# dkogan/horizonator

Hardware: AMD Instinct MI355X
Metric: panorama Mpix/s (360deg, 16k-wide, 7x7 SRTM3 tiles) (higher is better)
Workload: dtype f32

## Files before the change

### horizonator_amd/_lib.py

```python
import ctypes as C
import os

_HERE = os.path.dirname(os.path.abspath(__file__))
LIB_PATH = os.environ.get("HORIZONATOR_AMD_LIB") or os.path.join(_HERE, "libhorizonator.so")
DEMGEN_PATH = os.path.join(_HERE, "libhzdemgen.so")
SELFTEST_PATH = os.path.join(_HERE, "libhorizonator_selftest.so")

MAX_NDEMS_IJ = 4


class DemContext(C.Structure):
    _fields_ = [
        ("dems", (C.c_void_p * MAX_NDEMS_IJ) * MAX_NDEMS_IJ),
        ("mmap_sizes", (C.c_size_t * MAX_NDEMS_IJ) * MAX_NDEMS_IJ),
        ("mmap_fd", (C.c_int * MAX_NDEMS_IJ) * MAX_NDEMS_IJ),
        ("origin_dem_lon_lat", C.c_int * 2),
        ("origin_dem_cellij", C.c_int * 2),
        ("Ndems_ij", C.c_int * 2),
        ("radius_cells", C.c_int),
        ("cells_per_deg", C.c_int),
    ]


class _Offscreen(C.Structure):
# ... 166 lines not shown
    sig("hz_hip_last_times", i, vp, P(Times))
    sig("hz_hip_stream", vp, vp)
    sig("hz_hip_wait_outputs", i, vp, vp)
    sig("hz_hip_wait_for", i, vp, vp)
    sig("horizonator_amd_stream_waits_for_outputs", b, ctxp, vp)
    sig("horizonator_amd_waits_for_stream", b, ctxp, vp)
    sig("hz_hip_last_plan", i, vp, vp)
    sig("hz_hip_last_queue_counts", i, vp, vp)
    sig("hz_hip_last_error", C.c_char_p)
    if selftest:
        sig("hz_hip_check_fastmath", i, i, i, C.c_uint64, C.c_uint64, P(C.c_uint64), vp)
        sig("hz_hip_check_exactness", i, i, i, C.c_uint64, C.c_uint64, i, i, i, i, P(C.c_uint64))
        sig("hz_hip_debug_bigqueue", i, vp, i, vp, i, vp)
        sig("hz_hip_debug_wave_timing", i, vp, P(View), vp, C.c_size_t, vp)
        sig("hz_hip_debug_worklist", C.c_long, i, i, i, P(View), i, i, i, vp, C.c_size_t)
    return lib


DECLARED_SYMBOLS = [
    "horizonator_init", "horizonator_deinit", "horizonator_resized", "horizonator_pan_zoom",
    "horizonator_move", "horizonator_set_zextents", "horizonator_redraw", "horizonator_pick",
    "horizonator_render_offscreen", "horizonator_x_from_az", "horizonator_project",
    "horizonator_unproject",
    "horizonator_dem_init", "horizonator_dem_deinit", "horizonator_dem_sample",
    "horizonator_dem_bounds_latlon_deg",
    "horizonator_amd_get_window", "horizonator_amd_init_from_mosaic",
    "horizonator_amd_render", "horizonator_amd_render_device", "horizonator_amd_render_batch",
    "horizonator_amd_render_packed", "horizonator_amd_resolve_packed",
    "horizonator_amd_resolve_packed_strips", "horizonator_amd_render_sparse",
    "horizonator_amd_resolve_sparse_strips",
    "horizonator_amd_sync", "horizonator_amd_stream_waits_for_outputs", "horizonator_amd_waits_for_stream", "horizonator_amd_texture_layout", "horizonator_amd_set_texture",
    "horizonator_amd_set_sector", "horizonator_amd_set_raster", "horizonator_amd_set_profiling",
    "horizonator_amd_get_options", "horizonator_amd_set_options", "horizonator_amd_render_begin", "horizonator_amd_render_end",
    "horizonator_amd_last_times", "horizonator_amd_get_view", "horizonator_amd_device",
    "horizonator_amd_get_mosaic", "horizonator_amd_link_cells_size", "horizonator_amd_link_cells",
    "horizonator_amd_poi_visibility", "horizonator_amd_build_id",
    "hz_hip_device_count", "hz_hip_create", "hz_hip_destroy", "hz_hip_upload_mosaic",
    "hz_hip_download_mosaic", "hz_hip_ingest_tiles", "hz_hip_set_sector", "hz_hip_set_raster",
    "hz_hip_set_profiling", "hz_hip_get_options", "hz_hip_set_options", "hz_hip_set_texture", "hz_hip_pack", "hz_hip_resolve_packed", "hz_hip_pack_sparse", "hz_hip_resolve_sparse", "hz_hip_resolve_sparse_strips", "hz_hip_draw", "hz_hip_resolve", "hz_hip_resolve_to_host", "hz_hip_render_to_host", "hz_hip_host_begin", "hz_hip_host_end", "hz_hip_host_prepare",
    "hz_hip_read_depth", "hz_hip_link_cells", "hz_hip_poi_visibility", "hz_hip_sync", "hz_hip_last_times", "hz_hip_stream", "hz_hip_wait_outputs", "hz_hip_wait_for", "hz_hip_last_plan", "hz_hip_last_queue_counts", "hz_hip_last_error",
]
SELFTEST_SYMBOLS = ["hz_hip_check_fastmath", "hz_hip_check_exactness", "hz_hip_debug_bigqueue", "hz_hip_debug_wave_timing",
                    "hz_hip_debug_worklist"]


def load_demgen():
    if not os.path.exists(DEMGEN_PATH):
        raise ImportError(f"{DEMGEN_PATH} is missing: build it with `make -C horizonator_amd/csrc`")
    lib = C.CDLL(DEMGEN_PATH)
    lib.hz_demgen_write_region.restype = C.c_int
    lib.hz_demgen_write_region.argtypes = [C.c_char_p] + [C.c_int] * 6
    lib.hz_demgen_write_tile.restype = C.c_int
    lib.hz_demgen_write_tile.argtypes = [C.c_char_p] + [C.c_int] * 4
    lib.hz_demgen_tile_values.restype = None
    lib.hz_demgen_tile_values.argtypes = [C.c_void_p] + [C.c_int] * 4
    return lib
```

### horizonator_amd/csrc/hz_context.cpp

```cpp
#include "hz_dev.h"

#include <time.h>

thread_local char hz_g_last_error[512];
extern "C" const char* hz_hip_last_error(void) { return g_last_error; }


static int env_int(const char* name, int dflt) { const char* e = getenv(name); return e ? atoi(e) : dflt; }
static hz_options_t default_options(void)
{
    hz_options_t o;
    o.serial         = 0;
    o.rounds         = 0;
    o.near_cells     = -1;
    o.coarse_depth   = -1;
    o.tiles          = -1;
    o.tile_list      = 0;
    o.adapt          = 1;
    o.adapt_hi       = -1;
    o.pretest_march  = -1;
    o.worklists      = 1;
    o.fast_math      = 1;
    o.resolve_clears = 1;
    o.queue_capacity = 0;
// ... 54 lines not shown
    hz_device_guard device_guard_(d->device);
    (void)hz_sync_all(d);
    (void)hipFree(d->d_mosaic);
    for(int i=0; i<HZ_NFB; i++) { (void)hipFree(d->d_fbs[i]); (void)hipFree(d->d_touched[i]); }
    for(int i=0; i<2*HZ_NFB; i++)
    {
        (void)hipFree(d->d_bigrec_s[i]);
        (void)hipFree(d->d_bigitem_s[i]);
        (void)hipFree(d->d_midrec_s[i]);
        (void)hipFree(d->d_clip_s[i]);
        (void)hipFree(d->d_big_counters_s[i]);
        (void)hipFree(d->tiles_s[i].cursor); (void)hipFree(d->tiles_s[i].pairs); (void)hipFree(d->tiles_s[i].state); (void)hipFree(d->tiles_s[i].busy);
    }
    if(d->ev_marched) (void)hipEventDestroy(d->ev_marched);
    if(d->ev_near)    (void)hipEventDestroy(d->ev_near);
    for(int i=0; i<HZ_NFB; i++) (void)hipFree(d->d_hiz[i]);
    for(int c=0; c<HZ_LIST_CACHE; c++)
        for(int k=0; k<HZ_NLISTS; k++)
        {
            hz_worklists_t& wl = d->list_cache[c];
            (void)hipFree(wl.d_items[k]);
            for(int t=0; t<2; t++)
            {
                if(wl.h_items[k][t])   (void)hipHostFree(wl.h_items[k][t]);
                if(wl.ev_copied[k][t]) (void)hipEventDestroy(wl.ev_copied[k][t]);
            }
        }
    delete d->list_scratch; delete d->list_scratch2;
    (void)hipFree(d->d_texels);
    (void)hipFree(d->d_tanel);
// ... 93 lines not shown
        d->near_bigrec_capacity  = near_tris < rec ? (unsigned int)near_tris : rec;
        d->near_bigitem_capacity = 2*rec;
        d->near_clip_capacity    = d->near_bigrec_capacity;
        if(d->env.queue_capacity > 0)
            d->bigrec_capacity = d->bigitem_capacity = d->midrec_capacity = d->clip_capacity =
            d->near_bigrec_capacity = d->near_bigitem_capacity = d->near_clip_capacity = (unsigned int)d->env.queue_capacity;
    }
    if(d->env.serial) d->qstream = d->nstream = d->stream;
    else
    {
        HZ_CHECK(hipStreamCreateWithFlags(&d->qstream, hipStreamNonBlocking));
        HZ_CHECK(hipStreamCreateWithFlags(&d->nstream, hipStreamNonBlocking));
    }
    HZ_CHECK(hipEventCreateWithFlags(&d->ev_marched, hipEventDisableTiming));
    HZ_CHECK(hipEventCreateWithFlags(&d->ev_near,    hipEventDisableTiming));
    for(int i=0; i<2*HZ_NFB; i++)
    {
        const mr_queue_t q = hz_queue_set(d, i);
        HZ_CHECK(hipMalloc(&d->d_bigrec_s[i],  (size_t)q.bigrec_capacity*sizeof(hz_bigrec_t)));
        HZ_CHECK(hipMalloc(&d->d_bigitem_s[i], (size_t)q.bigitem_capacity*sizeof(hz_bigitem_t)));
        if(q.midrec_capacity) HZ_CHECK(hipMalloc(&d->d_midrec_s[i], (size_t)q.midrec_capacity*sizeof(hz_rec_t)));
        HZ_CHECK(hipMalloc(&d->d_clip_s[i],    (size_t)q.clip_capacity*sizeof(uint32_t)));
        HZ_CHECK(hipMalloc(&d->d_big_counters_s[i], HZ_NCOUNTERS*sizeof(unsigned int)));
        HZ_CHECK(hipMemset(d->d_big_counters_s[i], 0, HZ_NCOUNTERS*sizeof(unsigned int)));
        if(d->env.tiles > 0 && i >= HZ_NFB && hz_tile_bins(d, i) != 0) return -1;
    }
    sw.lap("queue sets");
    HZ_CHECK(hipEventRecord(d->ev_drawn, d->qstream));
    HZ_CHECK(hipMalloc(&d->d_tanel, (size_t)d->H*sizeof(float)));
    d->h_tanel = (float*)malloc((size_t)d->H*sizeof(float));
    d->tanel_resident = 0;
    for(int k=0; k<10; k++) HZ_CHECK(hipEventCreate(&d->ev[k]));
    for(int k=0; k<HZ_NFB; k++)
    {
        HZ_CHECK(hipHostMalloc((void**)&d->adapt.h_counts[k], 6*sizeof(unsigned int), hipHostMallocDefault));
        HZ_CHECK(hipEventCreateWithFlags(&d->adapt.ev[k], hipEventDisableTiming | hipEventReleaseToSystem));
    }
    sw.lap("the rest");
    return 0;
// ... 172 lines not shown
```

### horizonator_amd/csrc/hz_dev.h

```cpp
#pragma once

#include <hip/hip_runtime_api.h>

#include <math.h>
#include <stdio.h>
#include <stdlib.h>
#include <string.h>
#include <time.h>

#include <vector>

#include "hz_hip.h"
#include "hz_types.h"
#include "hz_launch.h"


extern thread_local char hz_g_last_error[512];
#define g_last_error hz_g_last_error

#define HZ_CHECK(call)                                                        \
    do {                                                                      \
        hipError_t e_ = (call);                                               \
        if(e_ != hipSuccess)                                                  \
        {                                                                     \
// ... 65 lines not shown
    std::vector<uint32_t>* list_scratch;
    std::vector<uint32_t>* list_scratch2;
    struct { unsigned long long* d_cycles; size_t capacity; unsigned int grid_x, grid_y; } wave_timing;

    hipStream_t stream, rstream;
    hipEvent_t  ev_drawn, ev_free[HZ_NFB], ev_readers, ev_tanel;
    int16_t*            d_mosaic;
    unsigned long long* d_fbs[HZ_NFB];
    size_t              fb_used[HZ_NFB];
    int                 fbi;
    unsigned long long* d_fb;
    unsigned char*      d_touched[HZ_NFB];
    int                 seg_stride;
    hipStream_t         qstream, nstream;
    hipEvent_t          ev_marched, ev_near;
    uint32_t*           d_hiz[HZ_NFB];
    int                 hiz_unavailable;
    int                 tiles_unavailable;
    struct
    {
        unsigned int* h_counts[HZ_NFB];
        hipEvent_t    ev[HZ_NFB];
        int           pending[HZ_NFB], long_of[HZ_NFB], reach_of[HZ_NFB];
        unsigned int  serial_of[HZ_NFB];
        hz_view_t     view; int col0, col1, have_view;
        unsigned int  serial;
        unsigned int  items_short;
        int           tried_long;
        int           long_reach;
        int           seen_reach; unsigned int seen_records, seen_items;
    } adapt;
    struct { hz_polar_t* d_polar; hz_xform_t key; int state ; int unavailable; hipEvent_t ev_filled;
             int same_draw;      } vc;
    int                 last_qshards_log2;
    int                 last_plan[5];
    int                 stream_reads_fb;
    hz_bigrec_t*        d_bigrec_s[2*HZ_NFB];
    hz_bigitem_t*       d_bigitem_s[2*HZ_NFB];
    hz_rec_t*           d_midrec_s[2*HZ_NFB];
    uint32_t*           d_clip_s[2*HZ_NFB];
    unsigned int*       d_big_counters_s[2*HZ_NFB];
    unsigned int        bigrec_capacity, bigitem_capacity, midrec_capacity, clip_capacity;
    unsigned int        near_bigrec_capacity, near_bigitem_capacity, near_clip_capacity;
    tl_bins_t           tiles_s[2*HZ_NFB];
    hz_view_t           last_view;
    int                 have_view;
    int                 fb_consumed;
    float*              d_tanel;
    float*              h_tanel;
    int                 tanel_resident;

    struct hz_hoststate* host;

    uint32_t*      d_texels;
    hz_texparams_t tex;
    int            tex_on;
// ... 49 lines not shown
```

### horizonator_amd/csrc/hz_draw.cpp

```cpp
#include "hz_dev.h"
#include "hz_fast.h"

static int upload_list(hz_dev_t* d, int which, hipStream_t st, const std::vector<uint32_t>& items)
{
    hz_worklists_t& wl = *d->lists;
    const size_t n = items.size();
    if(n > wl.cap[which])
    {
        HZ_CHECK(hz_sync_all(d));
        (void)hipFree(wl.d_items[which]); wl.d_items[which] = NULL;
        for(int t=0; t<2; t++) { if(wl.h_items[which][t]) (void)hipHostFree(wl.h_items[which][t]); wl.h_items[which][t] = NULL; }
        wl.cap[which] = 0;
        const size_t cap = n + n/4 + 1024;
        hipError_t e = hipMalloc(&wl.d_items[which], cap*sizeof(uint32_t));
        for(int t=0; t<2 && e == hipSuccess; t++) e = hipHostMalloc((void**)&wl.h_items[which][t], cap*sizeof(uint32_t), hipHostMallocDefault);
        if(e != hipSuccess)
        {
            (void)hipFree(wl.d_items[which]); wl.d_items[which] = NULL;
            for(int t=0; t<2; t++) { if(wl.h_items[which][t]) (void)hipHostFree(wl.h_items[which][t]); wl.h_items[which][t] = NULL; }
            HZ_CHECK(e);
        }
        wl.cap[which] = cap;
    }
    const int t = wl.turn[which]; wl.turn[which] ^= 1;
// ... 158 lines not shown
                return 0;
            }
            HZ_CHECK(hipEventCreateWithFlags(&d->vc.ev_filled, hipEventDisableTiming));
        }
        HZ_CHECK(hipStreamWaitEvent(d->nstream, d->ev_marched, 0));
        hzk_polar_fill(dim3((unsigned)((d->N + 255)/256), 1024), dim3(256), d->nstream, (const int16_t*)d->d_mosaic, d->vc.d_polar, d->N, p.u);
        HZ_CHECK(hipGetLastError());
        HZ_CHECK(hipEventRecord(d->vc.ev_filled, d->nstream));
        HZ_CHECK(hipStreamWaitEvent(d->stream, d->vc.ev_filled, 0));
        d->vc.state = 2;
    }
    p.vcache = d->vc.d_polar;
    return 0;
}

int hz_draw_impl(hz_dev_t* d, const hz_view_t* view)
{
    hz_params_t p = hz_make_params(d, view);
    const bool prof = d->profiling != 0;
    d->last_view = *view; d->have_view = 1; d->fb_consumed = 0;
    if(!d->adapt.have_view || memcmp(view, &d->adapt.view, sizeof(*view)) != 0 || d->adapt.col0 != d->col0 || d->adapt.col1 != d->col1)
    {
        d->adapt.view = *view; d->adapt.col0 = d->col0; d->adapt.col1 = d->col1; d->adapt.have_view = 1;
        d->adapt.serial++; d->adapt.items_short = 0; d->adapt.tried_long = 0; d->adapt.long_reach = 0;
    }
    for(int k=0; k<HZ_NFB; k++)
        if(d->adapt.pending[k] && hipEventQuery(d->adapt.ev[k]) == hipSuccess)
        {
            d->adapt.pending[k] = 0;
            const unsigned int items = d->adapt.h_counts[k][1];
// ... 51 lines not shown
            {
                hz_worklists_t* e = &d->list_cache[c];
                if(e->valid && memcmp(&key, &e->key, sizeof(key)) == 0) { hit = e; break; }
                if((!e->valid && lru->valid) || (e->valid == lru->valid && e->last_used < lru->last_used)) lru = e;
            }
            fresh_lists = hit == NULL;
            d->lists = hit ? hit : lru;
            d->lists->last_used = ++d->lists_clock;
            if(fresh_lists) { d->lists->valid = 0; d->lists->key = key; }
        }
        if(two_pass)
        {
            p.inline_max = HZ_INLINE_MAX_PIX;
            const mr_queue_t qn = hz_queue_set(d, HZ_NFB + next);
            HZ_CHECK(hipStreamWaitEvent(d->nstream, d->ev_free[next], 0));
            {
                const float ppr = p.halfW * p.u.az_ndc_per_rad;
                const float reach = 0.5f*(float)(p.near_j1 - p.near_j0);
                zoomed_view = reach > 0.f && ppr/reach >= HZ_HIZ_MIN_PX;
                const float cells_to_zfar = view->zfar / (p.u.deg_per_cell * 111194.9f);
                p.qshards_log2 = (zoomed_view || cells_to_zfar <= 0.25f*ppr) ? HZ_QSHARDS_LOG2 : 0;
            }
            hz_params_t p1 = p;
            p1.pass = 1; p1.early_z = 0;
            if(fresh_lists)
            {
                hz_list_rounds(p1, zn, a0, a1, false, d->list_scratch, *d->list_scratch2);
                if(upload_list(d, 0, d->nstream, *d->list_scratch) != 0) return -1;
            }
            if(prof) HZ_CHECK(hipEventRecord(d->ev[7], d->nstream));
// ... 24 lines not shown
                HZ_CHECK(hipStreamWaitEvent(d->stream, d->ev_near, 0));
                waited_near = true;
            }
            else
                near_beside_far = true;
            p.pass = 2; p.early_z = early_z ? 1 : 0;
            {
                const float ppr = p.halfW * p.u.az_ndc_per_rad;
                const float cells_to_zfar = view->zfar / (p.u.deg_per_cell * 111194.9f);
                if(cells_to_zfar <= 0.25f*ppr) p.inline_max = 32;
            }
            p.hiz = hz.l1;
            p.pretest_march = d->env.pretest_march >= 0 ? d->env.pretest_march
                                                        : ((unsigned long long)p.SW*(unsigned long long)p.H*8ull > (256ull << 20) ? 1 : 0);
        }
        else if(prof) { HZ_CHECK(hipEventRecord(d->ev[7], d->stream)); HZ_CHECK(hipEventRecord(d->ev[6], d->stream)); }
        if(!waited_near) HZ_CHECK(hipStreamWaitEvent(d->stream, d->ev_free[next], 0));
        if(fresh_lists)
        {
            if(!two_pass) hz_list_rounds(p, zn, a0, a1, true, NULL, *d->list_scratch2);
            if(upload_list(d, 1, d->stream, *d->list_scratch2) != 0) return -1;
            d->lists->valid = 1;
        }
        if(prof) HZ_CHECK(hipEventRecord(d->ev[9], d->stream));
        if(launch_march(d, d->stream, q, zn, p, listed ? d->lists->d_items[1] : NULL, d->lists->n[1]) != 0) return -1;
    }
    if(prof) HZ_CHECK(hipEventRecord(d->ev[2], d->stream));
    HZ_CHECK(hipEventRecord(d->ev_marched, d->stream));
    HZ_CHECK(hipStreamWaitEvent(d->qstream, d->ev_marched, 0));
    if(near_beside_far) HZ_CHECK(hipStreamWaitEvent(d->qstream, d->ev_near, 0));
    if(prof) HZ_CHECK(hipEventRecord(d->ev[8], d->qstream));
    unsigned int* report = NULL;
// ... 38 lines not shown
```

### horizonator_amd/csrc/hz_fast.h

```cpp
#pragma once

#include "hz_num.h"

#ifdef __HIPCC__

#define HZF_LO 9.31322575e-10f
#define HZF_HI 1073741824.0f

__device__ static inline int hzf_in_range(float x) { const float a = hz_abs(x); return a >= HZF_LO && a <= HZF_HI; }

__device__ static inline float hzf_refined_rcp(float c)
{
    const float r = __builtin_amdgcn_rcpf(c);
    const float e = __builtin_fmaf(-c, r, 1.0f);
    return __builtin_fmaf(e, r, r);
}
__device__ static inline float hzf_div_by(float a, float c, float rr)
{
    float q = a*rr;
    float e = __builtin_fmaf(-c, q, a);
    q = __builtin_fmaf(e, rr, q);
    e = __builtin_fmaf(-c, q, a);
    return __builtin_fmaf(e, rr, q);
}
// ... 51 lines not shown
    p = p + u7*-0.1173503194786851f;
    p = p + u9*0.0536813784310406f;
    p = p + (u9*-0.0121323213173444f)*u2;
    const float a   = (1.0f < tn) ? ((p*-2.0f + HZ_HALF_PI) + p) : p;
    const float arc = flip ? (HZ_HALF_PI + a) : a;
    const uint32_t sign = ((uint32_t)__float_as_int(y) | (uint32_t)__float_as_int(rcp)) & 0x80000000u;
    return __int_as_float((int)((uint32_t)__float_as_int(arc) | sign));
}
template<bool XPOS>
__device__ static inline float hzf_atan2(float y, float x)
{
    const float t = (XPOS ? false : (0.f >= x)) ? y : hz_abs(x);
    return hzf_atan2_r<XPOS>(y, x, hzf_rcp(t));
}

__device__ static inline hz_polar_t hzf_polar_en_r(const hz_xform_t* u, float e, float n, float fz, float rcp_az)
{
    hz_polar_t q;
    const float h = fz - u->viewer_z;
    const float nn = n*n, ee = e*e;
    q.d_ne  = hzf_sqrt(nn + ee);
    q.az    = hzf_atan2_r<false>(e, n, rcp_az);
    q.el    = hzf_atan2<true>(h, q.d_ne);
    q.d_enh = hzf_sqrt(h*h + nn + ee);
    return q;
}
__device__ static inline hz_polar_t hzf_polar_en(const hz_xform_t* u, float e, float n, float fz)
{
    return hzf_polar_en_r(u, e, n, fz, hzf_rcp((0.f >= n) ? e : hz_abs(n)));
}
__device__ static inline hz_vertex_t hzf_finish(const hz_xform_t* u, const hzf_const_t* c, hz_polar_t q)
{
    hz_vertex_t v;
    const float d = hzf_div_by_two_pi(q.az + -u->az_center, c->rr_two_pi);
    v.x = (HZ_TWO_PI*(d - hz_roundeven(d))) * u->az_ndc_per_rad;
    v.y = q.el * u->aspect * u->az_ndc_per_rad;
    v.z = hzf_div_by(q.d_enh - u->znear, c->zrange, c->rr_zrange) * 2.0f + -1.0f;

    const float r = hzf_div_by(q.d_ne - u->znear_color, c->crange, c->rr_crange);
    v.red = hz_min(hz_max(r, 0.0f), 1.0f);
    return v;
}
__device__ static inline hz_vertex_t hzf_transform_en(const hz_xform_t* u, const hzf_const_t* c, float e, float n, float fz)
{
    return hzf_finish(u, c, hzf_polar_en(u, e, n, fz));
}
__device__ static inline hz_vertex_t hzf_transform_en_r(const hz_xform_t* u, const hzf_const_t* c, float e, float n, float fz, float rcp_az)
{
    return hzf_finish(u, c, hzf_polar_en_r(u, e, n, fz, rcp_az));
}

#endif

HZ_HD int hzf_draw_ok(const hz_xform_t* u)
{
    const float lo = 9.31322575e-10f, hi = 1073741824.0f;
    const float vz = hz_abs(u->viewer_z), ce = hz_abs(u->az_center);
    const float zr = hz_abs(u->zfar - u->znear), cr = hz_abs(u->zfar_color - u->znear_color);
    if(!(vz == 0.0f || (vz >= 0.015625f && vz <= 536870912.0f))) return 0;
    if(!(ce == 0.0f || (ce >= 8.8817842e-16f && ce <= 1048576.0f))) return 0;
    if(!(u->znear >= lo && u->znear <= hi && hz_abs(u->zfar) >= lo && hz_abs(u->zfar) <= hi && zr >= lo && zr <= hi)) return 0;
    if(!(hz_abs(u->znear_color) >= lo && hz_abs(u->znear_color) <= hi &&
         hz_abs(u->zfar_color) >= lo && hz_abs(u->zfar_color) <= hi && cr >= lo && cr <= hi)) return 0;
    if(!(hz_abs(u->aspect) <= hi && hz_abs(u->az_ndc_per_rad) <= hi)) return 0;
    return 1;
// ... 2 lines not shown
```

### horizonator_amd/csrc/hz_k_march.h

```cpp
#pragma once


#define MR_CAP    128
#define MR_RSLOTS 4
#define MR_FIELDS 6

struct mr_lds_t
{
    uint32_t rows[MR_RSLOTS][MR_FIELDS][64];
    uint32_t ids[MR_CAP];
    uint32_t clip[64];
    uint32_t nclip;
};

__device__ static inline void mr_clip_flush(mr_lds_t& L, const mr_queue_t& q, int lane)
{
    const unsigned int nclip = (unsigned int)__builtin_amdgcn_readfirstlane((int)L.nclip);
    if(!nclip) return;
    uint32_t base = 0;
    if(lane == 0) base = atomicAdd(&q.counters[4], nclip);
    base = (uint32_t)__builtin_amdgcn_readfirstlane((int)base);
    if((unsigned int)lane < nclip)
    {
        const uint32_t at = base + (uint32_t)lane;
// ... 404 lines not shown
    }
    else { sx = (int)blockIdx.x + (p.pass == 1 ? p.near_x0 : 0); seg = (int)blockIdx.y; }
    const int i0   = sx*MR_COLS;
    const int i    = i0 + lane;
    int jbeg, jend;
    mr_segment_rows(zn, seg, &jbeg, &jend);
    if(p.pass)
    {
        const bool near = sx >= p.near_x0 && sx <= p.near_x1 && jbeg < p.near_j1 && jend > p.near_j0;
        if((p.pass == 1) != near) return;
    }
    const bool has_vertex = i < p.N;
    const bool has_cell   = lane < MR_COLS && i < p.N-1;
    const int  ic = has_vertex ? i : p.N-1;

    if(p.cull_strips)
    {
        const int ia = i0, ib = min(i0 + MR_COLS, p.N-1);
        const bool viewer_inside = p.u.viewer_cell_i >= (float)(ia-1) && p.u.viewer_cell_i <= (float)(ib+1) &&
                                   p.u.viewer_cell_j >= (float)(jbeg-1) && p.u.viewer_cell_j <= (float)(jend+1);
        if(!viewer_inside)
        {
            const hz_vertex_t v = hz_transform_en(&p.u, hz_east(&p.u, (float)((lane & 1) ? ib : ia)),
                                                  hz_north(&p.u, (float)((lane & 2) ? jend : jbeg)), 0.f);
            float xlo = 2.f, xhi = -2.f;
            #pragma unroll
            for(int c=0; c<4; c++)
            {
                const float xc = __builtin_bit_cast(float, __builtin_amdgcn_readlane(__builtin_bit_cast(int, v.x), c));
                xlo = hz_min(xlo, xc); xhi = hz_max(xhi, xc);
            }
            if(xhi - xlo <= 1.0f)
            {
                const float flo = (xlo*p.halfW + p.halfW) - 2.5f, fhi = (xhi*p.halfW + p.halfW) + 1.5f;
                if(fhi < (float)p.col0 || flo > (float)p.col1) return;
            }
        }
    }

    const float e = hz_east(&p.u, (float)ic);
    const float n_tab = hz_north(&p.u, (float)(jbeg + lane));
    auto north_of = [&](int rel) -> float
    {
        if(rel < 64) return __builtin_bit_cast(float, __builtin_amdgcn_readlane(__builtin_bit_cast(int, n_tab), rel));
        return hz_north(&p.u, (float)(jbeg + rel));
    };
    if(p.far_strips)
    {
        const int nrows = jend - jbeg;
        float nn = lane <= nrows ? n_tab*n_tab : __builtin_inff();
        if(nrows >= 64) { const float n64 = hz_north(&p.u, (float)(jbeg + 64)); nn = hz_min(nn, n64*n64); }
        #pragma unroll
        for(int m=32; m>=1; m>>=1) nn = hz_min(nn, __shfl_xor(nn, m));
        if(__all(nn + e*e > p.far_dd)) return;
    }

    const hzf_const_t fc = hzf_setup(&p.u);
    const bool fast_strip = p.fast_ok && __all(hzf_in_range(e));
    const unsigned long long fast_rows = __ballot(hzf_in_range(n_tab));
    const int  tab_rows   = min(jend - jbeg, 63);
    const bool rcp_south  = __all(lane > tab_rows || 0.f >= n_tab);
    const bool rcp_north  = __all(lane > tab_rows || !(0.f >= n_tab));
    const float rcp_tab   = VCACHE ? 0.f : hzf_rcp(rcp_south ? e : hz_abs(n_tab));

    unsigned int head = 0, count = 0;
    if(lane == 0) L.nclip = 0;
    __syncthreads();
    int first_row = 0;
    mr_rowstate_t prev = {};
    bool prev_simple = false;
    int16_t z_next = VCACHE ? (int16_t)0 : mosaic[(size_t)jbeg*p.N + ic];
    hz_polar_t q_next = {};
    if(VCACHE) q_next = p.vcache[(size_t)jbeg*p.N + ic];
    float n_cur = north_of(0);
    bool far_prev = true;
    bool far_cur  = __all(n_cur*n_cur + e*e > p.far_dd);
    for(int j = jbeg; j <= jend; j++)
    {
        const int rel = j - jbeg;
        const float z = (float)z_next;
        const hz_polar_t q_cur = q_next;
        if(j < jend)
        {
            if(VCACHE) q_next = p.vcache[(size_t)(j+1)*p.N + ic];
            else z_next = mosaic[(size_t)(j+1)*p.N + ic];
        }
        const float n_next   = (j == jend) ? 0.f : north_of(rel+1);
        const bool  far_next = (j == jend) || __all(n_next*n_next + e*e > p.far_dd);
        const bool  skip_row   = far_prev && far_cur && far_next;
        const bool  skip_cells = far_prev && far_cur;
        const float n = n_cur;
        n_cur = n_next; far_prev = far_cur; far_cur = far_next;
        if(skip_row) continue;

        const bool fast = fast_strip && (rel >= 64 ? hzf_in_range(n) : (int)((fast_rows >> rel) & 1ull));
        hz_vertex_t vtx;
        if(VCACHE) vtx = fast ? hzf_finish(&p.u, &fc, q_cur) : hz_finish(&p.u, q_cur);
        else if(fast)
        {
            float rcp_az;
            if(rel >= 64 || !(rcp_south || rcp_north)) rcp_az = hzf_rcp((0.f >= n) ? e : hz_abs(n));
            else if(rcp_south) rcp_az = rcp_tab;
            else rcp_az = __builtin_bit_cast(float, __builtin_amdgcn_readlane(__builtin_bit_cast(int, rcp_tab), rel));
            vtx = hzf_transform_en_r(&p.u, &fc, e, n, z, rcp_az);
#ifdef HZ_EXP_TRANSFORM_TWICE
            {
                float n2 = n; asm volatile("" : "+v"(n2));
                const hz_vertex_t v2 = hzf_transform_en_r(&p.u, &fc, e, n2, z, rcp_az);
                vtx.x = (v2.x == vtx.x) ? vtx.x : v2.y; vtx.y = (v2.y == vtx.y) ? vtx.y : v2.z;
                vtx.z = (v2.z == vtx.z) ? vtx.z : v2.x; vtx.red = (v2.red == vtx.red) ? vtx.red : v2.x;
            }
#endif
        }
        else vtx = hz_transform_en(&p.u, e, n, z);

        bool in_volume, in_guard;
        hz_wvert_t cur = mr_window(vtx, p, &in_volume, &in_guard);
        const bool cur_simple = __all(in_guard && in_volume);
        if(!cur_simple) mr_window_flags(cur, vtx, in_guard);

        if(count && first_row <= rel - MR_RSLOTS)
        {
            __syncthreads();
// ... 46 lines not shown
                    }
                    count += (unsigned int)__popcll(m);
                    if(count >= 64)
                    {
                        __syncthreads();
                        mr_flush<HIZ, SHARDS>(L, head, 64, lane, jbeg, i0, fb, q, p, dbg);
                        head = (head + 64) & (MR_CAP-1);
                        count -= 64;
                        if(count) first_row = (int)(L.ids[head] >> 7);
                        __syncthreads();
                    }
                }
            }
        }
        prev = now; prev_simple = cur_simple;
    }
    if(count)
    {
        __syncthreads();
        mr_flush<HIZ, SHARDS>(L, head, count, lane, jbeg, i0, fb, q, p, dbg);
    }
    mr_clip_flush(L, q, lane);
    if(COUNTERS && p.wave_cycles && lane == 0)
    {
        unsigned long long* o = &p.wave_cycles[((size_t)blockIdx.y*gridDim.x + blockIdx.x)*4];
        o[0] = __builtin_amdgcn_s_memtime() - t_start;
        o[1] = ((unsigned long long)dbgv[0] << 32) | dbgv[1];
        o[2] = ((unsigned long long)dbgv[2] << 32) | dbgv[3];
        o[3] = ((unsigned long long)dbgv[5] << 32) | dbgv[4];
    }
// ... 2 lines not shown
```

### horizonator_amd/csrc/hz_kernels.hip

```cpp
#include <hip/hip_runtime.h>

#include <math.h>
#include <stdio.h>
#include <stdlib.h>
#include <string.h>

#include "hz_hip.h"
#include "hz_types.h"
#include "hz_fast.h"

#include "hz_k_common.h"
#include "hz_k_hiz.h"
#include "hz_k_scatter.h"
#include "hz_k_tile.h"
#include "hz_k_march.h"
#include "hz_k_resolve.h"
#include "hz_k_tell.h"
#include "hz_k_tex.h"


__global__ __launch_bounds__(256)
void k_ingest(const unsigned char* const* __restrict__ tiles, int16_t* __restrict__ mosaic,
              int N, int ntx, int nty, int cpd, int oc_x, int oc_y)
{
    const int i = blockIdx.x*blockDim.x + threadIdx.x;
    const int j = blockIdx.y;
    if(i >= N) return;
    int cx = i + oc_x, tx = cx / cpd; cx -= tx*cpd; if(cx == 0 && tx > 0) { tx--; cx = cpd; }
    int cy = j + oc_y, ty = cy / cpd; cy -= ty*cpd; if(cy == 0 && ty > 0) { ty--; cy = cpd; }
// ... 136 lines not shown
    (void)counters;
    #define HZK_MARCH(H, V, S) hipLaunchKernelGGL((k_march<false, H, V, S>), grid, block, 0, stream, mosaic, fb, q, zn, p)
    if(shards)
    {
        if(vcache) { if(hiz) HZK_MARCH(true, true, true); else HZK_MARCH(false, true, true); }
        else       { if(hiz) HZK_MARCH(true, false, true); else HZK_MARCH(false, false, true); }
    }
    else
    {
        if(vcache) { if(hiz) HZK_MARCH(true, true, false); else HZK_MARCH(false, true, false); }
        else       { if(hiz) HZK_MARCH(true, false, false); else HZK_MARCH(false, false, false); }
    }
    #undef HZK_MARCH
}

void hzk_polar_fill(dim3 grid, dim3 block, hipStream_t stream, const int16_t* mosaic, hz_polar_t* q, int N, hz_xform_t u)
{
    hipLaunchKernelGGL(k_polar_fill, grid, block, 0, stream, mosaic, q, N, u);
}

void hzk_resolve(bool clear, dim3 grid, dim3 block, hipStream_t stream, unsigned long long* fb, const float* tanel, unsigned char* bgr, float* ranges, int32_t* index, uint32_t* z24, int SW, int H, float znear, float zfar, unsigned int* qa, unsigned int* qb)
{
    if(clear) hipLaunchKernelGGL(k_resolve<true>, grid, block, 0, stream, fb, tanel, bgr, ranges, index, z24, SW, H, znear, zfar, qa, qb);
    else hipLaunchKernelGGL(k_resolve<false>, grid, block, 0, stream, fb, tanel, bgr, ranges, index, z24, SW, H, znear, zfar, qa, qb);
}

void hzk_resolve4(bool clear, dim3 grid, dim3 block, hipStream_t stream, unsigned long long* fb, const float* tanel, unsigned char* bgr, float* ranges, int32_t* index, uint32_t* z24, int SW, int H, float znear, float zfar, unsigned char* touched, int seg_stride, unsigned int* qa, unsigned int* qb, int yo0, int yo1, int nt)
{
    if(clear) hipLaunchKernelGGL(k_resolve4<true>, grid, block, 0, stream, fb, tanel, bgr, ranges, index, z24, SW, H, znear, zfar, touched, seg_stride, qa, qb, yo0, yo1, nt);
    else hipLaunchKernelGGL(k_resolve4<false>, grid, block, 0, stream, fb, tanel, bgr, ranges, index, z24, SW, H, znear, zfar, touched, seg_stride, qa, qb, yo0, yo1, nt);
// ... 82 lines not shown
```

### horizonator_amd/csrc/hz_launch.h

```cpp
#pragma once

#include <hip/hip_runtime_api.h>

#include "hz_types.h"

void hzk_clip(bool wave_items, dim3 grid, dim3 block, hipStream_t stream, const int16_t* mosaic, unsigned long long* fb, mr_queue_t q, hz_params_t p);
void hzk_hiz(dim3 grid, dim3 block, hipStream_t stream, const unsigned long long* fb, const unsigned char* touched, int seg_stride, int SW, int H, hz_hiz_t hz, unsigned int nunits);
void hzk_mid(dim3 grid, dim3 block, hipStream_t stream, unsigned long long* fb, const hz_rec_t* midrec, const unsigned int* counters, unsigned int midrec_capacity, hz_params_t p);
void hzk_march(bool counters, bool hiz, bool vcache, dim3 grid, dim3 block, hipStream_t stream, const int16_t* mosaic, unsigned long long* fb, mr_queue_t q, mr_zones_t zn, hz_params_t p);
void hzk_resolve(bool clear, dim3 grid, dim3 block, hipStream_t stream, unsigned long long* fb, const float* tanel, unsigned char* bgr, float* ranges, int32_t* index, uint32_t* z24, int SW, int H, float znear, float zfar, unsigned int* qa, unsigned int* qb);
void hzk_resolve4(bool clear, dim3 grid, dim3 block, hipStream_t stream, unsigned long long* fb, const float* tanel, unsigned char* bgr, float* ranges, int32_t* index, uint32_t* z24, int SW, int H, float znear, float zfar, unsigned char* touched, int seg_stride, unsigned int* qa, unsigned int* qb, int yo0, int yo1, int nt);
void hzk_pack_host(bool clear, dim3 grid, dim3 block, hipStream_t stream, unsigned long long* fb, hz_hostpack_t o, int SW, int H, int col_off, unsigned char* touched, int seg_stride, unsigned int* qa, unsigned int* qb);
void hzk_tell(hipStream_t stream, hz_tell_t s);
void hzk_pack(bool clear, dim3 grid, dim3 block, hipStream_t stream, unsigned long long* fb, uint32_t* packed, int SW, int H, unsigned int* qa, unsigned int* qb);
void hzk_resolve_packed(dim3 grid, dim3 block, hipStream_t stream, const uint32_t* packed, int stride, int ncols, const float* tanel, unsigned char* bgr, float* ranges, int out_W, int out_col0, int H, float znear, float zfar);
void hzk_pack_sparse(bool clear, dim3 grid, dim3 block, hipStream_t stream, unsigned long long* fb, uint32_t* out, int SW, int H, int mask_stride, unsigned char* touched, int seg_stride, unsigned int* qa, unsigned int* qb);
void hzk_resolve_sparse(dim3 grid, dim3 block, hipStream_t stream, hz_strips_t st, int mask_stride, const float* tanel, unsigned char* bgr, float* ranges, int out_W, int H, float znear, float zfar);
void hzk_scatter(dim3 grid, dim3 block, hipStream_t stream, const int16_t* mosaic, unsigned long long* fb, mr_queue_t q, hz_params_t p);
void hzk_big(dim3 grid, dim3 block, hipStream_t stream, unsigned long long* fb, const hz_bigrec_t* bigrec, const hz_bigitem_t* bigitem, const unsigned int* big_counters, unsigned int bigrec_capacity, unsigned int bigitem_capacity, hz_params_t p, const unsigned int* tile_state, unsigned int* report);
void hzk_shade_tex(dim3 grid, dim3 block, hipStream_t stream, const unsigned long long* fb, const int16_t* mosaic, const uint32_t* texels, hz_texparams_t tp, unsigned char* bgr, hz_params_t p);
void hzk_tile_bin(dim3 grid, dim3 block, hipStream_t stream, const hz_bigrec_t* bigrec, const hz_bigitem_t* bigitem, const unsigned int* big_counters, unsigned int bigrec_capacity, tl_bins_t tb, hz_params_t p);
void hzk_tile_raster(dim3 grid, dim3 block, hipStream_t stream, unsigned long long* fb, const hz_bigrec_t* bigrec, tl_bins_t tb, hz_params_t p);
void hzk_ingest(dim3 grid, dim3 block, hipStream_t stream, const unsigned char* const* tiles, int16_t* mosaic, int N, int ntx, int nty, int cpd, int oc_x, int oc_y);
void hzk_link_cells(dim3 grid, dim3 block, hipStream_t stream, const unsigned long long* fb, const float* tanel, const float* sin_az, const float* cos_az, const double* cos_el, float* lat, float* lon, int W, int H, int cell_w, int cell_h, int nx, int ny, float znear, float zfar, double viewer_lat, double cos_viewer_lat, double viewer_lon);
void hzk_poi(dim3 grid, dim3 block, hipStream_t stream, const unsigned long long* fb, const float* tanel, const hz_poi_proj_t* proj, int npois, unsigned char* visible, float* label_x, float* label_y, int W, int H, int height_out, float znear, float zfar);
void hzk_polar_fill(dim3 grid, dim3 block, hipStream_t stream, const int16_t* mosaic, hz_polar_t* q, int N, hz_xform_t u);
```

### horizonator_amd/csrc/hz_selftest_impl.h

```cpp
#pragma once

__device__ static inline unsigned long long hz_mix64(unsigned long long x)
{
    x += 0x9E3779B97F4A7C15ull;
    x = (x ^ (x >> 30)) * 0xBF58476D1CE4E5B9ull;
    x = (x ^ (x >> 27)) * 0x94D049BB133111EBull;
    return x ^ (x >> 31);
}
__device__ static inline float hz_seeded_float(unsigned long long r, int elo, int ehi)
{
    const uint32_t mant = (uint32_t)r & 0x7FFFFFu, sign = (uint32_t)(r >> 23) & 1u;
    const uint32_t ex = (uint32_t)elo + (uint32_t)((r >> 24) % (unsigned long long)(ehi - elo + 1));
    return __uint_as_float((sign << 31) | (ex << 23) | mant);
}

__global__ __launch_bounds__(256)
void k_check_fastmath(int what, unsigned long long seed, unsigned long long n, unsigned long long* mismatches, float* first_bad)
{
    unsigned long long bad = 0;
    for(unsigned long long k = (unsigned long long)blockIdx.x*blockDim.x + threadIdx.x; k < n; k += (unsigned long long)gridDim.x*blockDim.x)
    {
        float a = 0.f, b = 0.f, want = 0.f, got = 0.f;
        bool in_range = true;
        if(what == 0)
// ... 401 lines not shown
    HZ_ON_DEVICE(d);
    HZ_CHECK(hz_sync_all(d));
    unsigned long long* d_cycles = NULL;
    HZ_CHECK(hipMalloc(&d_cycles, capacity_words*sizeof(unsigned long long)));
    HZ_CHECK(hipMemset(d_cycles, 0, capacity_words*sizeof(unsigned long long)));
    d->wave_timing.d_cycles = d_cycles; d->wave_timing.capacity = capacity_words;
    d->wave_timing.grid_x = d->wave_timing.grid_y = 0;
    int rc = hz_draw_impl(d, view);
    d->wave_timing.d_cycles = NULL; d->wave_timing.capacity = 0;
    if(rc == 0 && hz_sync_all(d) != hipSuccess) rc = -1;
    grid[0] = d->wave_timing.grid_x; grid[1] = d->wave_timing.grid_y;
    if(rc == 0 && hipMemcpy(out, d_cycles, (size_t)grid[0]*grid[1]*4*sizeof(unsigned long long), hipMemcpyDeviceToHost) != hipSuccess) rc = -1;
    (void)hipFree(d_cycles);
    return rc;
}
```

### horizonator_amd/csrc/hz_types.h

```cpp
#pragma once

#include <stddef.h>
#include <stdint.h>

#include "hz_raster.h"
#include "hz_tex.h"
#include "hz_scatter.h"


struct hz_hiz_t { uint32_t* l1; uint32_t* l2; int w1, w2; };

#define HZ_WHO_MARCH 0
#define HZ_WHO_BIG   1
#define HZ_WHO_OTHER 2

struct hz_params_t
{
    hz_xform_t u;
    float halfW, halfH;
    int   N;
    int   W, H;
    int   col0, col1;
    int   SW;
    unsigned long long* wave_cycles;
    unsigned int inline_max;
    unsigned int big_min;
    float far_dd;
    int   far_strips;
    const uint32_t* worklist;
    int   cull_strips;
    int   pass;
    int   near_x0, near_x1;
    int   near_j0, near_j1;
    int   early_z;
    int   pretest_march;
    int   qshards_log2;
#ifdef HZ_EXPERIMENTS
    int   exp_fb[2];
#endif
    const hz_polar_t* vcache;
    const uint32_t* hiz;
    float z_guard;
    float z_hide_k;
    int   fast_ok;
    int   quad_max_dx;
#ifdef HZ_EXPERIMENTS
    int   debug;
#endif
    unsigned char* touched;
    int   seg_stride;
};
#define HZ_SEG_LOG2 8
#define HZ_SEG      (1 << HZ_SEG_LOG2)

struct hz_rec_t
{
// ... 147 lines not shown
```

### include/hz_selftest.h

```cpp
#pragma once

#include "hz_hip.h"

#ifdef __cplusplus
extern "C" {
#endif

int  hz_hip_check_fastmath(int device, int what, unsigned long long seed, unsigned long long n,
                           unsigned long long* mismatches, float* first_bad);

int  hz_hip_check_exactness(int device, int what, unsigned long long seed, unsigned long long n,
                            int W, int H, int col0, int col1, unsigned long long* out);

int  hz_hip_debug_bigqueue(hz_dev_t* d, int set, unsigned int* counters, int max_rec, int32_t* recs);

long hz_hip_debug_worklist(int N, int W, int H, const hz_view_t* view, int col0, int col1, int round,
                           int32_t* out, size_t capacity_items);

int  hz_hip_debug_wave_timing(hz_dev_t* d, const hz_view_t* view, unsigned long long* out, size_t capacity_words, unsigned int* grid);

#ifdef __cplusplus
}
#endif
```

Before: 84610.

## Precompute per-row and per-column march tables in a separate kernel

Adds a small kernel on the near stream that precomputes, for every mosaic row and column, the north/east coordinate, its square, its reciprocal and range/south flags, plus the fast-math constants header. The marching kernel now reads these from constant-address-space loads instead of recomputing hz_north/hz_east, squares, reciprocals and ballots per strip and per row. The loads are forced into scalar registers. The cost is an extra kernel launch and event dependency per frame and extra table memory. Per-row scalar loads also replace the earlier readlane tricks.

Result: no change. 84780 (median of 4 runs) (+0.2%).

```diff
diff --git a/horizonator_amd/_lib.py b/horizonator_amd/_lib.py
--- a/horizonator_amd/_lib.py
+++ b/horizonator_amd/_lib.py
@@ -204,6 +204,7 @@
         sig("hz_hip_debug_bigqueue", i, vp, i, vp, i, vp)
         sig("hz_hip_debug_wave_timing", i, vp, P(View), vp, C.c_size_t, vp)
         sig("hz_hip_debug_worklist", C.c_long, i, i, i, P(View), i, i, i, vp, C.c_size_t)
+        sig("hz_hip_debug_march_tables", i, vp, i, vp)
     return lib
 
 
@@ -231,7 +232,7 @@
     "hz_hip_read_depth", "hz_hip_link_cells", "hz_hip_poi_visibility", "hz_hip_sync", "hz_hip_last_times", "hz_hip_stream", "hz_hip_wait_outputs", "hz_hip_wait_for", "hz_hip_last_plan", "hz_hip_last_queue_counts", "hz_hip_last_error",
 ]
 SELFTEST_SYMBOLS = ["hz_hip_check_fastmath", "hz_hip_check_exactness", "hz_hip_debug_bigqueue", "hz_hip_debug_wave_timing",
-                    "hz_hip_debug_worklist"]
+                    "hz_hip_debug_worklist", "hz_hip_debug_march_tables"]
 
 
 def load_demgen():
diff --git a/horizonator_amd/csrc/hz_context.cpp b/horizonator_amd/csrc/hz_context.cpp
--- a/horizonator_amd/csrc/hz_context.cpp
+++ b/horizonator_amd/csrc/hz_context.cpp
@@ -92,6 +92,8 @@
     }
     if(d->ev_marched) (void)hipEventDestroy(d->ev_marched);
     if(d->ev_near)    (void)hipEventDestroy(d->ev_near);
+    if(d->ev_tables)  (void)hipEventDestroy(d->ev_tables);
+    for(int i=0; i<HZ_NFB; i++) (void)hipFree(d->d_mtab_s[i]);
     for(int i=0; i<HZ_NFB; i++) (void)hipFree(d->d_hiz[i]);
     for(int c=0; c<HZ_LIST_CACHE; c++)
         for(int k=0; k<HZ_NLISTS; k++)
@@ -215,6 +217,7 @@
     }
     HZ_CHECK(hipEventCreateWithFlags(&d->ev_marched, hipEventDisableTiming));
     HZ_CHECK(hipEventCreateWithFlags(&d->ev_near,    hipEventDisableTiming));
+    HZ_CHECK(hipEventCreateWithFlags(&d->ev_tables,  hipEventDisableTiming));
     for(int i=0; i<2*HZ_NFB; i++)
     {
         const mr_queue_t q = hz_queue_set(d, i);
@@ -224,6 +227,7 @@
         HZ_CHECK(hipMalloc(&d->d_clip_s[i],    (size_t)q.clip_capacity*sizeof(uint32_t)));
         HZ_CHECK(hipMalloc(&d->d_big_counters_s[i], HZ_NCOUNTERS*sizeof(unsigned int)));
         HZ_CHECK(hipMemset(d->d_big_counters_s[i], 0, HZ_NCOUNTERS*sizeof(unsigned int)));
+        if(i < HZ_NFB) HZ_CHECK(hipMalloc(&d->d_mtab_s[i], HZ_MT_ENTRIES(d->N)*sizeof(hz_mt_entry_t)));
         if(d->env.tiles > 0 && i >= HZ_NFB && hz_tile_bins(d, i) != 0) return -1;
     }
     sw.lap("queue sets");
diff --git a/horizonator_amd/csrc/hz_dev.h b/horizonator_amd/csrc/hz_dev.h
--- a/horizonator_amd/csrc/hz_dev.h
+++ b/horizonator_amd/csrc/hz_dev.h
@@ -103,6 +103,7 @@
     int                 seg_stride;
     hipStream_t         qstream, nstream;
     hipEvent_t          ev_marched, ev_near;
+    hipEvent_t          ev_tables;
     uint32_t*           d_hiz[HZ_NFB];
     int                 hiz_unavailable;
     int                 tiles_unavailable;
@@ -129,6 +130,7 @@
     hz_rec_t*           d_midrec_s[2*HZ_NFB];
     uint32_t*           d_clip_s[2*HZ_NFB];
     unsigned int*       d_big_counters_s[2*HZ_NFB];
+    hz_mt_entry_t*      d_mtab_s[HZ_NFB];
     unsigned int        bigrec_capacity, bigitem_capacity, midrec_capacity, clip_capacity;
     unsigned int        near_bigrec_capacity, near_bigitem_capacity, near_clip_capacity;
     tl_bins_t           tiles_s[2*HZ_NFB];
diff --git a/horizonator_amd/csrc/hz_draw.cpp b/horizonator_amd/csrc/hz_draw.cpp
--- a/horizonator_amd/csrc/hz_draw.cpp
+++ b/horizonator_amd/csrc/hz_draw.cpp
@@ -196,6 +196,16 @@
     return 0;
 }
 
+static int march_tables(hz_dev_t* d, int next, bool nstream_waited_free, hz_params_t& p)
+{
+    if(!nstream_waited_free) HZ_CHECK(hipStreamWaitEvent(d->nstream, d->ev_free[next], 0));
+    hzk_march_tables(d->nstream, d->d_mtab_s[next], p.N, p.u);
+    HZ_CHECK(hipGetLastError());
+    HZ_CHECK(hipEventRecord(d->ev_tables, d->nstream));
+    p.mtab = d->d_mtab_s[next];
+    return 0;
+}
+
 int hz_draw_impl(hz_dev_t* d, const hz_view_t* view)
 {
     hz_params_t p = hz_make_params(d, view);
@@ -277,6 +287,7 @@
             p.inline_max = HZ_INLINE_MAX_PIX;
             const mr_queue_t qn = hz_queue_set(d, HZ_NFB + next);
             HZ_CHECK(hipStreamWaitEvent(d->nstream, d->ev_free[next], 0));
+            if(march_tables(d, next, true, p) != 0) return -1;
             {
                 const float ppr = p.halfW * p.u.az_ndc_per_rad;
                 const float reach = 0.5f*(float)(p.near_j1 - p.near_j0);
@@ -331,8 +342,12 @@
             p.pretest_march = d->env.pretest_march >= 0 ? d->env.pretest_march
                                                         : ((unsigned long long)p.SW*(unsigned long long)p.H*8ull > (256ull << 20) ? 1 : 0);
         }
-        else if(prof) { HZ_CHECK(hipEventRecord(d->ev[7], d->stream)); HZ_CHECK(hipEventRecord(d->ev[6], d->stream)); }
-        if(!waited_near) HZ_CHECK(hipStreamWaitEvent(d->stream, d->ev_free[next], 0));
+        else
+        {
+            if(march_tables(d, next, false, p) != 0) return -1;
+            if(prof) { HZ_CHECK(hipEventRecord(d->ev[7], d->stream)); HZ_CHECK(hipEventRecord(d->ev[6], d->stream)); }
+        }
+        if(!waited_near) HZ_CHECK(hipStreamWaitEvent(d->stream, d->ev_tables, 0));
         if(fresh_lists)
         {
             if(!two_pass) hz_list_rounds(p, zn, a0, a1, true, NULL, *d->list_scratch2);
diff --git a/horizonator_amd/csrc/hz_fast.h b/horizonator_amd/csrc/hz_fast.h
--- a/horizonator_amd/csrc/hz_fast.h
+++ b/horizonator_amd/csrc/hz_fast.h
@@ -89,16 +89,19 @@
     return hzf_atan2_r<XPOS>(y, x, hzf_rcp(t));
 }
 
-__device__ static inline hz_polar_t hzf_polar_en_r(const hz_xform_t* u, float e, float n, float fz, float rcp_az)
+__device__ static inline hz_polar_t hzf_polar_en_sq(const hz_xform_t* u, float e, float ee, float n, float nn, float fz, float rcp_az)
 {
     hz_polar_t q;
     const float h = fz - u->viewer_z;
-    const float nn = n*n, ee = e*e;
     q.d_ne  = hzf_sqrt(nn + ee);
     q.az    = hzf_atan2_r<false>(e, n, rcp_az);
     q.el    = hzf_atan2<true>(h, q.d_ne);
     q.d_enh = hzf_sqrt(h*h + nn + ee);
     return q;
+}
+__device__ static inline hz_polar_t hzf_polar_en_r(const hz_xform_t* u, float e, float n, float fz, float rcp_az)
+{
+    return hzf_polar_en_sq(u, e, e*e, n, n*n, fz, rcp_az);
 }
 __device__ static inline hz_polar_t hzf_polar_en(const hz_xform_t* u, float e, float n, float fz)
 {
@@ -124,6 +127,10 @@
 {
     return hzf_finish(u, c, hzf_polar_en_r(u, e, n, fz, rcp_az));
 }
+__device__ static inline hz_vertex_t hzf_transform_en_sq(const hz_xform_t* u, const hzf_const_t* c, float e, float ee, float n, float nn, float fz, float rcp_az)
+{
+    return hzf_finish(u, c, hzf_polar_en_sq(u, e, ee, n, nn, fz, rcp_az));
+}
 
 #endif
 
diff --git a/horizonator_amd/csrc/hz_k_march.h b/horizonator_amd/csrc/hz_k_march.h
--- a/horizonator_amd/csrc/hz_k_march.h
+++ b/horizonator_amd/csrc/hz_k_march.h
@@ -442,6 +442,9 @@
     const bool has_cell   = lane < MR_COLS && i < p.N-1;
     const int  ic = has_vertex ? i : p.N-1;
 
+    const hz_mt_entry_t* const rows_v = p.mtab + HZ_MT_HEAD;
+    const hz_mt_entry_t* const cols   = rows_v + p.N;
+
     if(p.cull_strips)
     {
         const int ia = i0, ib = min(i0 + MR_COLS, p.N-1);
@@ -449,8 +452,7 @@
                                    p.u.viewer_cell_j >= (float)(jbeg-1) && p.u.viewer_cell_j <= (float)(jend+1);
         if(!viewer_inside)
         {
-            const hz_vertex_t v = hz_transform_en(&p.u, hz_east(&p.u, (float)((lane & 1) ? ib : ia)),
-                                                  hz_north(&p.u, (float)((lane & 2) ? jend : jbeg)), 0.f);
+            const hz_vertex_t v = hz_transform_en(&p.u, cols[(lane & 1) ? ib : ia].v, rows_v[(lane & 2) ? jend : jbeg].v, 0.f);
             float xlo = 2.f, xhi = -2.f;
             #pragma unroll
             for(int c=0; c<4; c++)
@@ -466,30 +468,20 @@
         }
     }
 
-    const float e = hz_east(&p.u, (float)ic);
-    const float n_tab = hz_north(&p.u, (float)(jbeg + lane));
-    auto north_of = [&](int rel) -> float
-    {
-        if(rel < 64) return __builtin_bit_cast(float, __builtin_amdgcn_readlane(__builtin_bit_cast(int, n_tab), rel));
-        return hz_north(&p.u, (float)(jbeg + rel));
-    };
+    const hz_mt_entry_t col = cols[ic];
+    const float e = col.v, ee = col.vv;
     if(p.far_strips)
     {
         const int nrows = jend - jbeg;
-        float nn = lane <= nrows ? n_tab*n_tab : __builtin_inff();
-        if(nrows >= 64) { const float n64 = hz_north(&p.u, (float)(jbeg + 64)); nn = hz_min(nn, n64*n64); }
+        float nn = rows_v[min(jbeg + lane, jend)].vv;
+        if(nrows >= 64) nn = hz_min(nn, rows_v[jbeg + 64].vv);
         #pragma unroll
         for(int m=32; m>=1; m>>=1) nn = hz_min(nn, __shfl_xor(nn, m));
-        if(__all(nn + e*e > p.far_dd)) return;
-    }
-
-    const hzf_const_t fc = hzf_setup(&p.u);
-    const bool fast_strip = p.fast_ok && __all(hzf_in_range(e));
-    const unsigned long long fast_rows = __ballot(hzf_in_range(n_tab));
-    const int  tab_rows   = min(jend - jbeg, 63);
-    const bool rcp_south  = __all(lane > tab_rows || 0.f >= n_tab);
-    const bool rcp_north  = __all(lane > tab_rows || !(0.f >= n_tab));
-    const float rcp_tab   = VCACHE ? 0.f : hzf_rcp(rcp_south ? e : hz_abs(n_tab));
+        if(__all(nn + ee > p.far_dd)) return;
+    }
+
+    const hzf_const_t fc = mt_header(p);
+    const bool fast_strip = p.fast_ok && __all((col.flags & HZ_MT_IN_RANGE) != 0u);
 
     unsigned int head = 0, count = 0;
     if(lane == 0) L.nclip = 0;
@@ -500,9 +492,11 @@
     int16_t z_next = VCACHE ? (int16_t)0 : mosaic[(size_t)jbeg*p.N + ic];
     hz_polar_t q_next = {};
     if(VCACHE) q_next = p.vcache[(size_t)jbeg*p.N + ic];
-    float n_cur = north_of(0);
+    const mt_const_t rows = mt_rows(p);
+    hz_mt_entry_t r = mt_row(rows, jbeg);
+    asm volatile("" : "+s"(r.v), "+s"(r.vv), "+s"(r.rcp), "+s"(r.flags));
     bool far_prev = true;
-    bool far_cur  = __all(n_cur*n_cur + e*e > p.far_dd);
+    bool far_cur  = __all(r.vv + ee > p.far_dd);
     for(int j = jbeg; j <= jend; j++)
     {
         const int rel = j - jbeg;
@@ -513,28 +507,26 @@
             if(VCACHE) q_next = p.vcache[(size_t)(j+1)*p.N + ic];
             else z_next = mosaic[(size_t)(j+1)*p.N + ic];
         }
-        const float n_next   = (j == jend) ? 0.f : north_of(rel+1);
-        const bool  far_next = (j == jend) || __all(n_next*n_next + e*e > p.far_dd);
-        const bool  skip_row   = far_prev && far_cur && far_next;
+        const hz_mt_entry_t r_above = mt_row(rows, min(j + 1, jend));
         const bool  skip_cells = far_prev && far_cur;
-        const float n = n_cur;
-        n_cur = n_next; far_prev = far_cur; far_cur = far_next;
-        if(skip_row) continue;
-
-        const bool fast = fast_strip && (rel >= 64 ? hzf_in_range(n) : (int)((fast_rows >> rel) & 1ull));
+        if(skip_cells)
+        {
+            const bool far_next = (j == jend) || __all(r_above.vv + ee > p.far_dd);
+            if(far_next) { r = r_above; continue; }
+        }
+
+        const float n = r.v;
+        const bool fast = fast_strip && (r.flags & HZ_MT_IN_RANGE) != 0u;
         hz_vertex_t vtx;
         if(VCACHE) vtx = fast ? hzf_finish(&p.u, &fc, q_cur) : hz_finish(&p.u, q_cur);
         else if(fast)
         {
-            float rcp_az;
-            if(rel >= 64 || !(rcp_south || rcp_north)) rcp_az = hzf_rcp((0.f >= n) ? e : hz_abs(n));
-            else if(rcp_south) rcp_az = rcp_tab;
-            else rcp_az = __builtin_bit_cast(float, __builtin_amdgcn_readlane(__builtin_bit_cast(int, rcp_tab), rel));
-            vtx = hzf_transform_en_r(&p.u, &fc, e, n, z, rcp_az);
+            const float rcp_az = (r.flags & HZ_MT_SOUTH) ? col.rcp : r.rcp;
+            vtx = hzf_transform_en_sq(&p.u, &fc, e, ee, n, r.vv, z, rcp_az);
 #ifdef HZ_EXP_TRANSFORM_TWICE
             {
                 float n2 = n; asm volatile("" : "+v"(n2));
-                const hz_vertex_t v2 = hzf_transform_en_r(&p.u, &fc, e, n2, z, rcp_az);
+                const hz_vertex_t v2 = hzf_transform_en_sq(&p.u, &fc, e, ee, n2, r.vv, z, rcp_az);
                 vtx.x = (v2.x == vtx.x) ? vtx.x : v2.y; vtx.y = (v2.y == vtx.y) ? vtx.y : v2.z;
                 vtx.z = (v2.z == vtx.z) ? vtx.z : v2.x; vtx.red = (v2.red == vtx.red) ? vtx.red : v2.x;
             }
@@ -611,6 +603,9 @@
             }
         }
         prev = now; prev_simple = cur_simple;
+        far_prev = far_cur;
+        far_cur  = (j == jend) || __all(r_above.vv + ee > p.far_dd);
+        r = r_above;
     }
     if(count)
     {
diff --git a/horizonator_amd/csrc/hz_k_tables.h b/horizonator_amd/csrc/hz_k_tables.h
--- /dev/null
+++ b/horizonator_amd/csrc/hz_k_tables.h
@@ -0,0 +1,50 @@
+#pragma once
+
+__global__ __launch_bounds__(256)
+void k_march_tables(hz_mt_entry_t* __restrict__ t, int N, hz_xform_t u)
+{
+    const int k = (int)(blockIdx.x*blockDim.x + threadIdx.x);
+    if(k < N)
+    {
+        hz_mt_entry_t r;
+        r.v = hz_north(&u, (float)k);
+        r.vv = r.v*r.v;
+        r.rcp = hzf_rcp(hz_abs(r.v));
+        r.flags = (hzf_in_range(r.v) ? HZ_MT_IN_RANGE : 0u) | ((0.f >= r.v) ? HZ_MT_SOUTH : 0u);
+        t[HZ_MT_HEAD + k] = r;
+    }
+    else if(k < 2*N)
+    {
+        hz_mt_entry_t c;
+        c.v = hz_east(&u, (float)(k - N));
+        c.vv = c.v*c.v;
+        c.rcp = hzf_rcp(c.v);
+        c.flags = hzf_in_range(c.v) ? HZ_MT_IN_RANGE : 0u;
+        t[HZ_MT_HEAD + k] = c;
+    }
+    else if(k == 2*N)
+    {
+        const hzf_const_t fc = hzf_setup(&u);
+        hz_mt_entry_t h0, h1;
+        h0.v = fc.rr_two_pi; h0.vv = fc.rr_zrange; h0.rcp = fc.rr_crange; h0.flags = __float_as_uint(fc.zrange);
+        h1.v = fc.crange; h1.vv = 0.f; h1.rcp = 0.f; h1.flags = 0u;
+        t[0] = h0; t[1] = h1;
+    }
+}
+
+typedef const __attribute__((address_space(4))) hz_mt_entry_t* mt_const_t;
+__device__ static inline mt_const_t mt_rows(const hz_params_t& p) { return (mt_const_t)(uintptr_t)(p.mtab + HZ_MT_HEAD); }
+__device__ static inline hz_mt_entry_t mt_row(mt_const_t rows, int j)
+{
+    hz_mt_entry_t r;
+    r.v = rows[j].v; r.vv = rows[j].vv; r.rcp = rows[j].rcp; r.flags = rows[j].flags;
+    return r;
+}
+__device__ static inline hzf_const_t mt_header(const hz_params_t& p)
+{
+    const mt_const_t h = (mt_const_t)(uintptr_t)p.mtab;
+    hzf_const_t fc;
+    fc.rr_two_pi = h[0].v; fc.rr_zrange = h[0].vv; fc.rr_crange = h[0].rcp; fc.zrange = __uint_as_float(h[0].flags);
+    fc.crange = h[1].v;
+    return fc;
+}
diff --git a/horizonator_amd/csrc/hz_kernels.hip b/horizonator_amd/csrc/hz_kernels.hip
--- a/horizonator_amd/csrc/hz_kernels.hip
+++ b/horizonator_amd/csrc/hz_kernels.hip
@@ -13,6 +13,7 @@
 #include "hz_k_hiz.h"
 #include "hz_k_scatter.h"
 #include "hz_k_tile.h"
+#include "hz_k_tables.h"
 #include "hz_k_march.h"
 #include "hz_k_resolve.h"
 #include "hz_k_tell.h"
@@ -179,6 +180,11 @@
     #undef HZK_MARCH
 }
 
+void hzk_march_tables(hipStream_t stream, hz_mt_entry_t* t, int N, hz_xform_t u)
+{
+    hipLaunchKernelGGL(k_march_tables, dim3((unsigned)((2*N + 1 + 255)/256)), dim3(256), 0, stream, t, N, u);
+}
+
 void hzk_polar_fill(dim3 grid, dim3 block, hipStream_t stream, const int16_t* mosaic, hz_polar_t* q, int N, hz_xform_t u)
 {
     hipLaunchKernelGGL(k_polar_fill, grid, block, 0, stream, mosaic, q, N, u);
diff --git a/horizonator_amd/csrc/hz_launch.h b/horizonator_amd/csrc/hz_launch.h
--- a/horizonator_amd/csrc/hz_launch.h
+++ b/horizonator_amd/csrc/hz_launch.h
@@ -24,4 +24,5 @@
 void hzk_ingest(dim3 grid, dim3 block, hipStream_t stream, const unsigned char* const* tiles, int16_t* mosaic, int N, int ntx, int nty, int cpd, int oc_x, int oc_y);
 void hzk_link_cells(dim3 grid, dim3 block, hipStream_t stream, const unsigned long long* fb, const float* tanel, const float* sin_az, const float* cos_az, const double* cos_el, float* lat, float* lon, int W, int H, int cell_w, int cell_h, int nx, int ny, float znear, float zfar, double viewer_lat, double cos_viewer_lat, double viewer_lon);
 void hzk_poi(dim3 grid, dim3 block, hipStream_t stream, const unsigned long long* fb, const float* tanel, const hz_poi_proj_t* proj, int npois, unsigned char* visible, float* label_x, float* label_y, int W, int H, int height_out, float znear, float zfar);
+void hzk_march_tables(hipStream_t stream, hz_mt_entry_t* t, int N, hz_xform_t u);
 void hzk_polar_fill(dim3 grid, dim3 block, hipStream_t stream, const int16_t* mosaic, hz_polar_t* q, int N, hz_xform_t u);
diff --git a/horizonator_amd/csrc/hz_selftest_impl.h b/horizonator_amd/csrc/hz_selftest_impl.h
--- a/horizonator_amd/csrc/hz_selftest_impl.h
+++ b/horizonator_amd/csrc/hz_selftest_impl.h
@@ -439,3 +439,59 @@
     (void)hipFree(d_cycles);
     return rc;
 }
+
+
+__global__ __launch_bounds__(64)
+void k_check_tables(hz_mt_entry_t* __restrict__ t, int N, hz_xform_t u)
+{
+    const int lane = threadIdx.x, first = (int)blockIdx.x*64, k = first + lane;
+    hz_mt_entry_t o;
+    if(blockIdx.y == 0)
+    {
+        const float n_tab = hz_north(&u, (float)(first + lane));
+        const unsigned long long fast_rows = __ballot(hzf_in_range(n_tab));
+        o.v = n_tab; o.vv = n_tab*n_tab; o.rcp = hzf_rcp(hz_abs(n_tab));
+        o.flags = (((fast_rows >> lane) & 1ull) ? HZ_MT_IN_RANGE : 0u) | ((0.f >= n_tab) ? HZ_MT_SOUTH : 0u);
+        if(k < N) t[HZ_MT_HEAD + k] = o;
+    }
+    else
+    {
+        const float e = hz_east(&u, (float)k);
+        o.v = e; o.vv = e*e; o.rcp = hzf_rcp(e); o.flags = hzf_in_range(e) ? HZ_MT_IN_RANGE : 0u;
+        if(k < N) t[HZ_MT_HEAD + N + k] = o;
+    }
+    if(blockIdx.x == 0 && blockIdx.y == 0 && lane == 0)
+    {
+        const hzf_const_t fc = hzf_setup(&u);
+        hz_mt_entry_t h0, h1;
+        h0.v = fc.rr_two_pi; h0.vv = fc.rr_zrange; h0.rcp = fc.rr_crange; h0.flags = __float_as_uint(fc.zrange);
+        h1.v = fc.crange; h1.vv = 0.f; h1.rcp = 0.f; h1.flags = 0u;
+        t[0] = h0; t[1] = h1;
+    }
+}
+
+extern "C" int hz_hip_debug_march_tables(hz_dev_t* d, int which, uint32_t* out)
+{
+    HZ_ON_DEVICE(d);
+    if(which < 0 || which > 1 || !out || !d->have_view || d->raster == HZ_RASTER_SCATTER)
+    {
+        snprintf(g_last_error, sizeof(g_last_error), "hz_hip_debug_march_tables: bad arguments, or the last draw was not the marching kernel's");
+        return -1;
+    }
+    HZ_CHECK(hz_sync_all(d));
+    const size_t bytes = HZ_MT_ENTRIES(d->N)*sizeof(hz_mt_entry_t);
+    if(which == 0)
+    {
+        HZ_CHECK(hipMemcpy(out, d->d_mtab_s[d->fbi], bytes, hipMemcpyDeviceToHost));
+        return 0;
+    }
+    const hz_params_t p = hz_make_params(d, &d->last_view);
+    hz_mt_entry_t* t = NULL;
+    HZ_CHECK(hipMalloc(&t, bytes));
+    hipLaunchKernelGGL(k_check_tables, dim3((unsigned)((d->N + 63)/64), 2), dim3(64), 0, 0, t, d->N, p.u);
+    hipError_t e = hipGetLastError();
+    if(e == hipSuccess) e = hipMemcpy(out, t, bytes, hipMemcpyDeviceToHost);
+    (void)hipFree(t);
+    HZ_CHECK(e);
+    return 0;
+}
diff --git a/horizonator_amd/csrc/hz_types.h b/horizonator_amd/csrc/hz_types.h
--- a/horizonator_amd/csrc/hz_types.h
+++ b/horizonator_amd/csrc/hz_types.h
@@ -13,6 +13,12 @@
 #define HZ_WHO_MARCH 0
 #define HZ_WHO_BIG   1
 #define HZ_WHO_OTHER 2
+
+struct hz_mt_entry_t { float v, vv, rcp; uint32_t flags; };
+#define HZ_MT_IN_RANGE 1u
+#define HZ_MT_SOUTH    2u
+#define HZ_MT_HEAD     2
+#define HZ_MT_ENTRIES(N) ((size_t)HZ_MT_HEAD + 2*(size_t)(N))
 
 struct hz_params_t
 {
@@ -40,6 +46,7 @@
 #endif
     const hz_polar_t* vcache;
     const uint32_t* hiz;
+    const hz_mt_entry_t* mtab;
     float z_guard;
     float z_hide_k;
     int   fast_ok;
diff --git a/include/hz_selftest.h b/include/hz_selftest.h
--- a/include/hz_selftest.h
+++ b/include/hz_selftest.h
@@ -19,6 +19,8 @@
 
 int  hz_hip_debug_wave_timing(hz_dev_t* d, const hz_view_t* view, unsigned long long* out, size_t capacity_words, unsigned int* grid);
 
+int  hz_hip_debug_march_tables(hz_dev_t* d, int which, uint32_t* out);
+
 #ifdef __cplusplus
 }
 #endif
```
